# adobe/3D-FM-GAN

Hardware: AMD Instinct MI355X
Metric: (photo,render) pairs/sec (higher is better)
Workload: dtype f32; 1 GPU; pairs1024: cfg4 shard: E_Tsr+E_W+E_W_Plus(18 styles) on 256^2 -> co-mod -> Generator(1024) forward, fp32, B=8/GPU; pairs_per_gpu=8, global_pairs=8, image_size=1024, parallelism=replicas x1 (batch-sharded, no collective), launch=eager, ranks=1, full=False

## Files before the change

3d-fm-gan_amd/op/_native.py:

```python
import ctypes
import os

import torch

_HERE = os.path.dirname(os.path.abspath(__file__))
LIB_PATH = os.environ.get('FMGAN_LIB') or os.path.join(os.path.dirname(_HERE), 'csrc', 'libfmgan_hip.so')

F32, F64, F16 = 0, 1, 2
FMGAN_OK, FMGAN_EUNSUPPORTED = 0, -2
_DTYPES = {torch.float32: F32, torch.float64: F64, torch.float16: F16}

_lib = None

amp_fwd = torch.amp.custom_fwd(device_type='cuda', cast_inputs=torch.float32)
amp_bwd = torch.amp.custom_bwd(device_type='cuda')


def _sig(fn, argtypes, restype=ctypes.c_int):
    fn.argtypes = argtypes
    fn.restype = restype
    return fn


def lib():
    global _lib
    if _lib is not None:
        return _lib
    if not os.path.exists(LIB_PATH):
        raise RuntimeError(
            f'{LIB_PATH} not found: the HIP extension is not built. Run `make -C {os.path.dirname(LIB_PATH)}` '
            f'(or __graft_entry__.build()). There is no CPU or PyTorch fallback for these ops.')
    L = ctypes.CDLL(LIB_PATH)
    vp, i, f, ll = ctypes.c_void_p, ctypes.c_int, ctypes.c_float, ctypes.c_longlong
    _sig(L.fmgan_abi_version, [])
    _sig(L.fmgan_status_string, [i], ctypes.c_char_p)
    _sig(L.fmgan_upfirdn2d_select, [i] * 15)
    _sig(L.fmgan_upfirdn2d_out_size, [i] * 12 + [ctypes.POINTER(i)] * 2)
    _sig(L.fmgan_upfirdn2d, [i, vp, vp, vp] + [i] * 15 + [vp])
    _sig(L.fmgan_upfirdn2d_strided, [i, vp, vp, vp] + [i] * 4 + [ll, i] + [i] * 11 + [vp])
    _sig(L.fmgan_blur_noise_bias_act_f32, [vp] * 3 + [i] * 4 + [ll, i] + [i] * 6 + [vp] * 3 + [i, f, f, vp])
    _sig(L.fmgan_blur_noise_bias_act_select, [vp] * 3 + [i] * 4 + [ll, i] + [i] * 6)
    _sig(L.fmgan_blur_noise_bias_act_path_f32, [vp] * 3 + [i] * 4 + [ll, i] + [i] * 6 + [vp] * 3 + [i, f, f, i, vp])
    _sig(L.fmgan_fused_bias_act, [i, vp, vp, vp, vp, ll, i, i, i, i, f, f, vp])
    _sig(L.fmgan_noise_bias_act_f32, [vp] * 5 + [i] * 4 + [f, f, vp])
    _sig(L.fmgan_fused_bias_act_bwd_blocks, [ll, i])
    _sig(L.fmgan_fused_bias_act_bwd_f32, [vp] * 4 + [ll, i, f, f, vp])
    _sig(L.fmgan_prelu_backward_blocks, [ll, i])
    _sig(L.fmgan_prelu_backward_f32, [vp] * 5 + [ll, i, vp])
    _sig(L.fmgan_face_region_blocks, [i, ll])
    _sig(L.fmgan_face_region_loss_f32, [vp] * 3 + [i, i, ll, vp])
    _sig(L.fmgan_face_region_backward_f32, [vp] * 4 + [i, i, ll, vp])
    _sig(L.fmgan_render_mask_f32, [vp] * 2 + [i, i, ll, vp])
    _sig(L.fmgan_face_input_blocks, [i] * 4)
    _sig(L.fmgan_face_input_f32, [vp] * 5 + [i] * 4 + [vp])
    _sig(L.fmgan_lpips_pair_input_select, [i] * 8)
    _sig(L.fmgan_lpips_pair_input_f32, [vp] * 5 + [i] * 8 + [vp])
    _sig(L.fmgan_projection_loss_select, [i] * 4)
    _sig(L.fmgan_projection_loss_blocks, [i] * 4)
    _sig(L.fmgan_projection_loss_fwd_f32, [vp] * 7 + [i] * 4 + [vp])
    _sig(L.fmgan_projection_loss_bwd_f32, [vp] * 7 + [i] * 4 + [vp])
    _sig(L.fmgan_lpips_distance_blocks, [i] * 3)
    _sig(L.fmgan_lpips_distance_f32, [vp] * 4 + [i, i, i, f, vp])
    _sig(L.fmgan_lpips_distance_backward_f32, [vp] * 6 + [i, i, i, f, vp])
    _sig(L.fmgan_bn_prelu_f32, [vp] * 5 + [f, vp, vp] + [vp] * 4 + [f, vp, vp] + [i] * 5 + [vp])
    _sig(L.fmgan_se_pool_chunks, [i] * 4)
    _sig(L.fmgan_se_pool_f32, [vp, vp] + [i] * 4 + [vp])
    _sig(L.fmgan_se_gate_f32, [vp, i, ll] + [vp] * 4 + [f] + [vp] * 3 + [i] * 3 + [vp])
    _sig(L.fmgan_ir_tail_f32, [vp] * 5 + [f, vp, vp] + [i] * 3 + [vp] * 4 + [f, vp] + [vp] * 4 + [f, vp] + [i] * 4 + [vp])
    _sig(L.fmgan_modconv_demod_f32, [vp] * 3 + [i] * 4 + [f, f, vp])
    _sig(L.fmgan_modconv_wsq_f32, [vp] * 2 + [i] * 3 + [vp])
    _sig(L.fmgan_modconv_demod_wsq_f32, [vp] * 3 + [i] * 3 + [f, f, vp])
    _sig(L.fmgan_equal_linear_f32, [vp] * 4 + [i] * 3 + [vp])
    _sig(L.fmgan_wino_weight_f32, [vp, vp, i, i, vp])
    _sig(L.fmgan_wino_input_f32, [vp] * 3 + [i] * 4 + [vp])
    _sig(L.fmgan_wino_output_f32, [vp] * 6 + [i] * 6 + [f, f, vp])
    _sig(L.fmgan_modconv_weight_prep_f32, [vp, vp, i, i, i, f, i, vp])
    _sig(L.fmgan_modconv2d_workspace_bytes, [i] * 6, ll)
    _sig(L.fmgan_modconv2d_f32, [vp] * 5 + [i] * 6 + [vp] * 3 + [i, i, f, f, ll, i, vp, ll, vp])
    _sig(L.fmgan_modconv_weight_bf16_bytes, [i] * 3, ll)
    _sig(L.fmgan_modconv_weight_to_bf16, [vp, vp, i, i, i, vp])
    _sig(L.fmgan_modconv2d_bf16_supported, [i] * 6)
    _sig(L.fmgan_modconv2d_bf16, [vp] * 5 + [i] * 6 + [vp] * 3 + [i, i, f, f, ll, i, vp])
    _sig(L.fmgan_modconv_weight_bf16x3_bytes, [i] * 3, ll)
    _sig(L.fmgan_modconv_weight_to_bf16x3, [vp, vp, i, i, i, vp])
    _sig(L.fmgan_modconv2d_bf16x3_supported, [i] * 6)
    _sig(L.fmgan_modconv2d_bf16x3, [vp] * 5 + [i] * 6 + [vp] * 3 + [i, i, f, f, ll, i, vp])
    _sig(L.fmgan_modconv2d_rgb_fusable, [i] * 5)
    _sig(L.fmgan_modconv2d_select, [i] * 8 + [ctypes.POINTER(i)] * 5)
    _sig(L.fmgan_modconv2d_tiles, [ctypes.POINTER(i), i])
    _sig(L.fmgan_torgb_weight_mod_f32, [vp] * 3 + [i] * 3 + [f, vp])
    _sig(L.fmgan_modconv2d_rgb_f32, [vp] * 5 + [i] * 5 + [vp] * 3 + [i, i, f, f] + [vp] * 4 + [i, vp])
    _sig(L.fmgan_modconv_wgrad_workspace_bytes, [i] * 5, ll)
    _sig(L.fmgan_modconv_wgrad_f32, [vp] * 5 + [i] * 5 + [f, vp, ll, vp])
    _sig(L.fmgan_modconv_wgrad_mode_workspace_bytes, [i] * 6, ll)
    _sig(L.fmgan_modconv_wgrad_mode_f32, [vp] * 5 + [i] * 6 + [f, vp, ll, vp])
    _sig(L.fmgan_images_to_tensor, [vp, vp, i, i, i, f, f, vp])
    _sig(L.fmgan_resize_output_size, [i, i, i, ctypes.POINTER(ctypes.c_int), ctypes.POINTER(ctypes.c_int)])
    _sig(L.fmgan_resize_plan_ints, [i] * 4, ll)
    _sig(L.fmgan_resize_plan, [i] * 4 + [vp, ll])
    _sig(L.fmgan_resize_bilinear_u8, [vp] * 4 + [i] * 5 + [f, f, vp])
    _sig(L.fmgan_tensor_to_images, [vp, vp, i, i, i, f, f, vp])
    _sig(L.fmgan_torgb_f32, [vp] * 6 + [i] * 4 + [f, vp])
    _sig(L.fmgan_torgb_backward_splits, [i] * 3)
    _sig(L.fmgan_torgb_backward_f32, [vp] * 6 + [i] * 4 + [f, vp])
    _sig(L.fmgan_refresh_entry_bytes, [])
    _sig(L.fmgan_weight_refresh_blocks, [i, i, i, i, ll], ll)
    _sig(L.fmgan_weight_refresh_f32, [vp, i, ll, vp])
    _sig(L.fmgan_style_bank_entry_bytes, [])
    _sig(L.fmgan_style_bank_f32, [vp, i, vp, vp, i, i, i, vp, vp])
    _sig(L.fmgan_demod_bank_f32, [vp, i, vp, i, vp, vp])
    if L.fmgan_abi_version() != 1:
        raise RuntimeError('libfmgan_hip.so ABI version mismatch')
    _lib = L
    return L


def check(status, what):
    if status != FMGAN_OK:
        raise RuntimeError(f'{what}: {lib().fmgan_status_string(status).decode()} (status {status})')


def served(status, what):
    if status == FMGAN_EUNSUPPORTED:
        return False
    check(status, what)
    return True


def require_gpu(t, name):
    if not t.is_cuda:
        raise RuntimeError(f'{name} must be a CUDA tensor (this build has no CPU path)')


def dtype_code(t):
    try:
        return _DTYPES[t.dtype]
    except KeyError:
        raise RuntimeError(f'unsupported dtype {t.dtype}: float32/float64/float16 only') from None


def ptr(t):
    return None if t is None else t.data_ptr()


def fp(t):
    if t is None:
        return None
    if t.dtype != torch.float32 or not t.is_cuda:
        raise RuntimeError(f'libfmgan_hip f32 entry point got a {t.dtype} tensor on {t.device}: float32 GPU tensors only '
                           f'(cast before the call; under autocast the package\'s autograd Functions do)')
    return t.data_ptr()


class on_device:

    def __init__(self, t):
        self.dev = t.device
        self.guard = None

    def __enter__(self):
        if torch.cuda.current_device() != self.dev.index:
            self.guard = torch.cuda.device(self.dev)
            self.guard.__enter__()
        return torch.cuda.current_stream(self.dev).cuda_stream

    def __exit__(self, *exc):
        if self.guard is not None:
            self.guard.__exit__(*exc)
        return False


BLUR_PATHS = {}


class _NullObserver:
    wants_paths = False

    def begin(self, name, info):
        return None

    def end(self, token):
        pass


_observer = _NullObserver()


def set_observer(obs=None):
    global _observer
    _observer = obs if obs is not None else _NullObserver()


class launching(on_device):

    def __init__(self, t, name, info):
        on_device.__init__(self, t)
        self.name, self.info = name, info

    def __enter__(self):
        stream = on_device.__enter__(self)
        self.tok = _observer.begin(self.name, self.info)
        return stream

    def __exit__(self, *exc):
        if exc[0] is None:
            _observer.end(self.tok)
        return on_device.__exit__(self, *exc)


def _noise_args(noise):
    if noise is None:
        return None, 1
    nz = noise.contiguous()
    return nz, nz.shape[0]


def upfirdn2d_out_size(in_h, in_w, kh, kw, up_x, up_y, down_x, down_y, px0, px1, py0, py1):
    oh, ow = ctypes.c_int(), ctypes.c_int()
    check(lib().fmgan_upfirdn2d_out_size(in_h, in_w, kh, kw, up_x, up_y, down_x, down_y, px0, px1, py0, py1,
                                         ctypes.byref(oh), ctypes.byref(ow)), 'upfirdn2d_out_size')
    return oh.value, ow.value
# ... 264 lines not shown

def projection_loss_bwd(x, target, mask, g_y, k, scale):
    b, h, w, f = _projection_loss_args(x, target, mask, (scale,))
    if k.numel() != 1 or k.device != x.device:
        raise ValueError(f'projection_loss_bwd: k must hold one element on x\'s device, got {tuple(k.shape)} on {k.device}')
    if g_y is not None:
        if tuple(g_y.shape) != (b, 3, 256, 256) or not nhwc_dense(g_y) or g_y.device != x.device:
            raise ValueError(f'projection_loss_bwd: g_y {tuple(g_y.shape)} with strides {g_y.stride()}: expected '
                             f'[{b}, 3, 256, 256] in channels_last storage on x\'s device')
    pk, pg = fp(k), fp(g_y)
    if b == 0 or lib().fmgan_projection_loss_select(b, h, w, f) <= 0:
        return None
    with launching(x, 'projection_loss', (b, h, f, mask is not None, g_y is not None, 1)) as stream:
        grad_x = torch.empty_like(x)
        st = lib().fmgan_projection_loss_bwd_f32(fp(x), fp(target), fp(mask), pg, pk, fp(scale), fp(grad_x), b, h, w, f,
                                                 stream)
    return grad_x if served(st, 'projection_loss_bwd') else None


def nhwc_dense(t):
    return t.ndim == 4 and t.permute(0, 2, 3, 1).is_contiguous()


def _lpips_distance_shape(f0, f1, w):
    if f0.ndim != 4 or tuple(f0.shape) != tuple(f1.shape) or w.numel() != f0.shape[1]:
        raise ValueError(f'lpips_distance: features {tuple(f0.shape)} and {tuple(f1.shape)}, weight {tuple(w.shape)}: '
                         f'expected two [N, C, H, W] tensors of one shape and C weights')
    if not (nhwc_dense(f0) and nhwc_dense(f1)):
        raise ValueError('lpips_distance: features must be NHWC-dense (channels_last storage); the kernel reads a '
                         'pixel\'s channel vector as one contiguous run')
    n, c, h, wd = f0.shape
    return n, c, h * wd


def lpips_distance(f0, f1, w, eps=1e-10):
    n, c, hw = _lpips_distance_shape(f0, f1, w)
    w = w.contiguous()
    p0, p1, pw = fp(f0), fp(f1), fp(w)
    if n == 0:
        return torch.zeros((0,), dtype=torch.float32, device=f0.device)
    blocks = lib().fmgan_lpips_distance_blocks(n, c, hw)
    if blocks <= 0:
        return None
    partial = torch.empty((n, blocks), dtype=torch.float32, device=f0.device)
    with launching(f0, 'lpips_distance', (n, c, hw, 0)) as stream:
        st = lib().fmgan_lpips_distance_f32(p0, p1, pw, fp(partial), n, c, hw, float(eps), stream)
    return partial.sum(1) / hw if served(st, 'lpips_distance') else None


def lpips_distance_backward(f0, f1, w, grad, need0, need1, eps=1e-10):
    n, c, hw = _lpips_distance_shape(f0, f1, w)
    if not (need0 or need1):
        return None, None
    gl = grad.reshape(-1)
    if gl.numel() != n:
        raise ValueError(f'lpips_distance_backward: grad must hold one element per sample ({n}), got {tuple(grad.shape)}')
    gl = gl.to(device=f0.device, dtype=torch.float32).contiguous()
    w = w.contiguous()
    p0, p1, pw, pg = fp(f0), fp(f1), fp(w), fp(gl)
    g0 = torch.empty_like(f0) if need0 else None
    g1 = torch.empty_like(f1) if need1 else None
    if n == 0:
        return g0, g1
    with launching(f0, 'lpips_distance', (n, c, hw, 1)) as stream:
        st = lib().fmgan_lpips_distance_backward_f32(p0, p1, pw, pg, fp(g0), fp(g1), n, c, hw, float(eps), stream)
    return (g0, g1) if served(st, 'lpips_distance_backward') else None


def _nhwc(t, name):
    require_gpu(t, name)
    fp(t)
    if not nhwc_dense(t):
        raise RuntimeError(f'{name}: expected a [B,C,H,W] tensor in channels_last storage, got {tuple(t.shape)} with '
                           f'strides {t.stride()}')
    return tuple(t.shape)


def _bn_args(bn, c):
    if bn is None:
        return None, None, None, None, 0.0
    mean, var, gamma, beta, eps = bn
    vs = [v.contiguous() for v in (mean, var, gamma, beta)]
    if any(v.numel() != c for v in vs):
        raise ValueError(f'BatchNorm vectors must hold {c} elements, got {[v.numel() for v in vs]}')
    return fp(vs[0]), fp(vs[1]), fp(vs[2]), fp(vs[3]), float(eps)


def _nhwc_empty(b, c, h, w, device):
    return torch.empty((b, c, h, w), dtype=torch.float32, device=device, memory_format=torch.channels_last)


def bn_prelu(x, bn, slope, want_y=True, bn_next=None, sub_stride=0):
    b, c, h, w = _nhwc(x, 'bn_prelu input')
    if not (want_y or bn_next is not None or sub_stride >= 1):
        raise ValueError('bn_prelu: no output requested')
    slope = slope.contiguous()
    if slope.numel() != c:
        raise ValueError(f'bn_prelu: {slope.numel()} slopes for {c} channels')
    y = torch.empty_like(x) if want_y else None
    y_next = torch.empty_like(x) if bn_next is not None else None
    y_sub = None
    if sub_stride >= 1:
        y_sub = _nhwc_empty(b, c, (h - 1) // sub_stride + 1, (w - 1) // sub_stride + 1, x.device)
    with launching(x, 'bn_prelu', (b, c, h, w)) as stream:
        st = lib().fmgan_bn_prelu_f32(fp(x), *_bn_args(bn, c), fp(slope), fp(y), *_bn_args(bn_next, c), fp(y_next),
                                      fp(y_sub), b, c, h, w, max(int(sub_stride), 0), stream)
    return (y, y_next, y_sub) if served(st, 'bn_prelu') else None


def se_pool(r):
    b, c, h, w = _nhwc(r, 'se_pool input')
    chunks = lib().fmgan_se_pool_chunks(b, c, h, w)
    if chunks <= 0:
        return None
    partial = torch.empty((b, chunks, c), dtype=torch.float32, device=r.device)
    with launching(r, 'se_pool', (b, c, h, w)) as stream:
        st = lib().fmgan_se_pool_f32(fp(r), fp(partial), b, c, h, w, stream)
    return partial if served(st, 'se_pool') else None


def se_gate(partial, hw, bn, fc1, fc2):
    require_gpu(partial, 'se_gate partials')
    b, chunks, c = partial.shape
    mid = fc1.shape[0]
    if tuple(fc1.shape[:2]) != (mid, c) or tuple(fc2.shape[:2]) != (c, mid) or fc1.numel() != mid * c \
            or fc2.numel() != mid * c:
        raise ValueError(f'se_gate: fc1 {tuple(fc1.shape)} / fc2 {tuple(fc2.shape)} do not fit {c} channels')
    fc1, fc2, partial = fc1.reshape(mid, c).contiguous(), fc2.reshape(c, mid).contiguous(), partial.contiguous()
    gate = torch.empty((b, c), dtype=torch.float32, device=partial.device)
    with launching(partial, 'se_gate', (b, c, mid, chunks)) as stream:
        st = lib().fmgan_se_gate_f32(fp(partial), chunks, int(hw), *_bn_args(bn, c), fp(fc1), fp(fc2), fp(gate), b, c,
                                     mid, stream)
    return gate if served(st, 'se_gate') else None


def ir_tail(r, bn, gate, shortcut, sc_stride=1, bn_sc=None, bn_next=None):
    b, c, h, w = _nhwc(r, 'ir_tail input')
    sb, scc, sh, sw = _nhwc(shortcut, 'ir_tail shortcut')
    exp = (h, w) if bn_sc is not None else ((sh - 1) // sc_stride + 1, (sw - 1) // sc_stride + 1)
    if (sb, scc) != (b, c) or exp != (h, w) or (bn_sc is not None and ((sh, sw) != (h, w) or sc_stride != 1)):
        raise ValueError(f'ir_tail: shortcut {tuple(shortcut.shape)} at stride {sc_stride} does not cover {tuple(r.shape)}')
    if gate is not None:
        if tuple(gate.shape) != (b, c):
            raise ValueError(f'ir_tail: gate {tuple(gate.shape)} for {tuple(r.shape)}')
        gate = gate.contiguous()
    out = torch.empty_like(r)
    out_next = torch.empty_like(r) if bn_next is not None else None
    with launching(r, 'ir_tail', (b, c, h, w, sc_stride, bn_sc is not None)) as stream:
        st = lib().fmgan_ir_tail_f32(fp(r), *_bn_args(bn, c), fp(gate), fp(shortcut), sh, sw, int(sc_stride),
                                     *_bn_args(bn_sc, c), fp(out), *_bn_args(bn_next, c), fp(out_next), b, c, h, w, stream)
    return (out, out_next) if served(st, 'ir_tail') else None


def modconv_demod(weight, style, scale, eps=1e-8, wsq=None):
    cout, cin, kh, kw = weight.shape[-4:]
    style = style.contiguous()
    demod = torch.empty((style.shape[0], cout), dtype=torch.float32, device=style.device)
    with on_device(style) as stream:
        if wsq is not None:
            check(lib().fmgan_modconv_demod_wsq_f32(fp(wsq), fp(style), fp(demod), style.shape[0], cout, cin,
                                                    float(scale), float(eps), stream), 'modconv_demod_wsq')
        else:
            check(lib().fmgan_modconv_demod_f32(fp(weight), fp(style), fp(demod), style.shape[0], cout, cin,
                                                kh * kw, float(scale), float(eps), stream), 'modconv_demod')
    return demod


def equal_linear(x, weight, bias=None):
    require_gpu(x, 'input')
    x, weight = x.contiguous(), weight.contiguous()
    b, k = x.shape
    n = weight.shape[0]
    if weight.shape[1] != k:
        raise RuntimeError(f'equal_linear: weight {tuple(weight.shape)} does not match input {tuple(x.shape)}')
    out = torch.empty((b, n), dtype=torch.float32, device=x.device)
    with on_device(x) as stream:
        check(lib().fmgan_equal_linear_f32(fp(x), fp(weight), fp(bias), fp(out), b, n, k, stream), 'equal_linear')
    return out


def style_bank(table, n_entries, w, wplus, styles_out):
    if w.dim() != 2 or wplus.dim() != 3 or wplus.shape[2] != w.shape[1] or not (w.is_contiguous() and wplus.is_contiguous()):
        raise RuntimeError(f'style_bank: W {tuple(w.shape)} / W+ {tuple(wplus.shape)} must be contiguous [T,D] / [P,n,D]')
    with on_device(w) as stream:
        check(lib().fmgan_style_bank_f32(fp(table.view(torch.float32)), n_entries, fp(w), fp(wplus), wplus.shape[0],
                                         w.shape[0], w.shape[1], fp(styles_out), stream), 'style_bank')


def demod_bank(table, n_entries, styles, batch, demod_out):
    with on_device(styles) as stream:
        check(lib().fmgan_demod_bank_f32(fp(table.view(torch.float32)), n_entries, fp(styles), batch, fp(demod_out), stream),
              'demod_bank')


def modconv_wsq(weight):
    cout, cin, kh, kw = weight.shape[-4:]
    wsq = torch.empty((cout, cin), dtype=torch.float32, device=weight.device)
    with on_device(weight) as stream:
        check(lib().fmgan_modconv_wsq_f32(fp(weight), fp(wsq), cout, cin, kh * kw, stream), 'modconv_wsq')
    return wsq


def modconv_weight_prep(weight, scale, kind=0):
    cout, cin, kh, kw = weight.shape[-4:]
    shape = (cin, kh * kw, cout) if kind == 0 else (cout, kh * kw, cin)
    wt = torch.empty(shape, dtype=torch.float32, device=weight.device)
    with on_device(weight) as stream:
        check(lib().fmgan_modconv_weight_prep_f32(fp(weight), fp(wt), cout, cin, kh * kw, float(scale), int(kind),
                                                  stream), 'modconv_weight_prep')
    return wt


def aligned_rows_shape(b, c, oh, ow, pad0):
    off = pad0 % 4
    rs = (ow + off + 31) // 32 * 32
    return (b * c, oh, rs), off, oh * rs, rs


def aligned_rows_buffer(b, c, oh, ow, pad0, device):
    shape, off, ps, rs = aligned_rows_shape(b, c, oh, ow, pad0)
    buf = torch.empty(shape, dtype=torch.float32, device=device)
    return buf, buf.data_ptr() + 4 * off, ps, rs


_mc_precision = 'f32'


class modconv_precision:

    def __init__(self, precision):
        if precision not in ('f32', 'bf16', 'bf16x3'):
            raise ValueError("precision must be 'f32', 'bf16' or 'bf16x3'")
        self.precision = precision

    def __enter__(self):
        global _mc_precision
        self.prev, _mc_precision = _mc_precision, self.precision
        return self

    def __exit__(self, *exc):
        global _mc_precision
        _mc_precision = self.prev
        return False


def modconv_weight_to_bf16(wt):
    cin, taps, cout = wt.shape
    nbytes = lib().fmgan_modconv_weight_bf16_bytes(cin, cout, taps)
    wtb = torch.empty(nbytes // 2, dtype=torch.int16, device=wt.device)
    with on_device(wt) as stream:
        check(lib().fmgan_modconv_weight_to_bf16(fp(wt), ptr(wtb), cin, cout, taps, stream), 'modconv_weight_to_bf16')
    return wtb


def wino_weight(wt):
    cin, taps, cout = wt.shape
    if taps != 9:
        raise RuntimeError('wino_weight: 3x3 weights only')
    u = torch.empty((16, cout, cin), dtype=torch.float32, device=wt.device)
    with on_device(wt) as stream:
        check(lib().fmgan_wino_weight_f32(fp(wt), fp(u), cin, cout, stream), 'wino_weight')
    return u


def wino_input(x, style):
    require_gpu(x, 'input')
    x, style = x.contiguous(), style.contiguous()
    b, cin, h, w = x.shape
    v = torch.empty((16, cin, b * (h // 2) * (w // 2)), dtype=torch.float32, device=x.device)
    with on_device(x) as stream:
        check(lib().fmgan_wino_input_f32(fp(x), fp(style), fp(v), b, cin, h, w, stream), 'wino_input')
    return v


def wino_output(m, demod, batch, h, w, noise=None, noise_weight=None, bias=None, fuse_act=False, alpha=0.2,
                act_scale=2 ** 0.5):
    require_gpu(m, 'm')
    m = m.contiguous()
    cout = m.shape[1]
    if m.shape[0] != 16 or m.shape[2] != batch * (h // 2) * (w // 2):
        raise RuntimeError('wino_output: M must be [16, cout, B*(H/2)*(W/2)]')
    out = torch.empty((batch, cout, h, w), dtype=torch.float32, device=m.device)
    nz, nb = _noise_args(noise)
    with on_device(m) as stream:
        check(lib().fmgan_wino_output_f32(fp(m), fp(demod), fp(nz), fp(noise_weight), fp(bias), fp(out), batch, cout, h, w,
                                          nb, int(bool(fuse_act)), float(alpha), float(act_scale), stream), 'wino_output')
    return out


def modconv2d_winograd(x, wt, style, demod, noise=None, noise_weight=None, bias=None, fuse_act=False, alpha=0.2,
                       act_scale=2 ** 0.5, u=None):
    require_gpu(x, 'input')
    x, style = x.contiguous(), style.contiguous()
    b, cin, h, w = x.shape
    if (h | w) & 1:
        raise RuntimeError('modconv2d_winograd: H and W must be even')
    if u is None:
        u = wino_weight(wt)
    cout = u.shape[1]
    n = b * (h // 2) * (w // 2)
    v = torch.empty((16, cin, n), dtype=torch.float32, device=x.device)
    m = torch.empty((16, cout, n), dtype=torch.float32, device=x.device)
    out = torch.empty((b, cout, h, w), dtype=torch.float32, device=x.device)
    nz, nb = _noise_args(noise)
    with launching(x, 'modconv2d_winograd', (b, cin, cout, h, w, 0)) as stream:
        check(lib().fmgan_wino_input_f32(fp(x), fp(style), fp(v), b, cin, h, w, stream), 'wino_input')
# ... 215 lines not shown
```

3d-fm-gan_amd/psp_encoder_model/encoders/psp_encoders.py:

```python
import math
import os

import torch
import torch.nn.functional as F
from torch import nn
from torch.nn import BatchNorm2d, Conv2d, Module, Sequential

from . import helpers
from .helpers import PReLU, bottleneck_IR, bottleneck_IR_SE, get_blocks
from stylegan2 import EqualLinear
from op import fused_leaky_relu
from op.live_weights import LiveWeights
from Util.streams import overlap_ok, run_deferred, side_streams

HEAD_STREAMS = int(os.environ.get('FMGAN_PSP_STREAMS', '2'))
GROUP_HEADS = os.environ.get('FMGAN_PSP_GROUPED', '0') == '1'

_TAPS = {18: (3, 5, 7), 50: (6, 20, 23)}


class GradualStyleBlock(Module):

    def __init__(self, in_c, out_c, spatial):
        super().__init__()
        self.out_c = out_c
        self.spatial = spatial
        layers, c = [], in_c
        for _ in range(int(math.log2(spatial))):
            layers += [Conv2d(c, out_c, kernel_size=3, stride=2, padding=1), nn.LeakyReLU()]
            c = out_c
        self.convs = nn.Sequential(*layers)
        self.linear = EqualLinear(out_c, out_c, lr_mul=1)

    def forward(self, x):
        if x.is_cuda and x.dtype == torch.float32:
            for conv, act in zip(self.convs[0::2], self.convs[1::2]):
                y = F.conv2d(x, conv.weight, None, conv.stride, conv.padding)
                if y.is_contiguous(memory_format=torch.channels_last) and not y.is_contiguous():
                    n, c, h, w = y.shape
                    y = fused_leaky_relu(y.permute(0, 2, 3, 1).reshape(-1, c), conv.bias, act.negative_slope, 1.0)
                    x = y.view(n, h, w, c).permute(0, 3, 1, 2)
                else:
                    x = fused_leaky_relu(y, conv.bias, act.negative_slope, 1.0)
            return self.linear(x.reshape(-1, self.out_c))
        return self.linear(self.convs(x).reshape(-1, self.out_c))


class GradualStyleEncoder(Module):
    def __init__(self, num_layers, mode='ir', opts=None):
        super().__init__()
        assert num_layers in [18, 50, 100, 152], 'num_layers should be 18, 50, 100, or 152'
        assert mode in ['ir', 'ir_se'], 'mode should be ir or ir_se'
        self.num_layers = num_layers
        unit = bottleneck_IR if mode == 'ir' else bottleneck_IR_SE
        self.input_layer = Sequential(Conv2d(opts.input_nc, 64, (3, 3), 1, 1, bias=False), BatchNorm2d(64), PReLU(64))
        self.body = Sequential(*[unit(b.in_channel, b.depth, b.stride) for stage in get_blocks(num_layers) for b in stage])
        self.style_count = opts.n_styles
        self.coarse_ind = 3
        self.middle_ind = 7
        self.styles = nn.ModuleList()
        for i in range(self.style_count):
            spatial = 16 if i < self.coarse_ind else (32 if i < self.middle_ind else 64)
            self.styles.append(GradualStyleBlock(512, 512, spatial))
        self.latlayer1 = nn.Conv2d(256, 512, kernel_size=1, stride=1, padding=0)
        self.latlayer2 = nn.Conv2d(128, 512, kernel_size=1, stride=1, padding=0)
        self.channels_last = True
        self._cl_key = None
        self._live_weights = None
        self._flat = None

    def _to_channels_last(self):
        w = self.input_layer[0].weight
        key = (w.device, w.data_ptr())
        if self._cl_key != key:
            for m in self.modules():
                if isinstance(m, nn.Conv2d):
                    m.weight.data = m.weight.data.contiguous(memory_format=torch.channels_last)
            self._cl_key = (w.device, self.input_layer[0].weight.data_ptr())

    def _levels(self):
        n = self.style_count
        return [list(range(0, min(self.coarse_ind, n))), list(range(self.coarse_ind, min(self.middle_ind, n))),
                list(range(self.middle_ind, n))]

    def _flatten_heads(self):
        def aliased(big, parts):
            step = big[0:parts[0].shape[0]].numel() * big.element_size()
            return all(q.data_ptr() == big.data_ptr() + g * step and q.stride() == big[0:q.shape[0]].stride()
                       for g, q in enumerate(parts))
        if self._flat is not None and all(aliased(wb, [self.styles[j].convs[2 * d].weight for j in idxs]) and
                                          aliased(bb, [self.styles[j].convs[2 * d].bias for j in idxs])
                                          for idxs, per_depth in self._flat for d, (wb, bb) in enumerate(per_depth)):
            return self._flat
        flat = []
        with torch.no_grad():
            for idxs in self._levels():
                if not idxs:
                    continue
                per_depth = []
                for d in range(len(self.styles[idxs[0]].convs) // 2):
                    convs = [self.styles[j].convs[2 * d] for j in idxs]
                    wb = torch.cat([c.weight.data for c in convs], 0)
                    if convs[0].weight.data.is_contiguous(memory_format=torch.channels_last) and wb.dim() == 4:
                        wb = wb.contiguous(memory_format=torch.channels_last)
                    bb = torch.cat([c.bias.data for c in convs], 0)
                    co = convs[0].weight.shape[0]
                    for g, c in enumerate(convs):
                        c.weight.data = wb[g * co:(g + 1) * co]
                        c.bias.data = bb[g * co:(g + 1) * co]
                    per_depth.append((wb, bb))
                flat.append((idxs, per_depth))
        self._flat = flat
        return flat

    def _grouped_heads(self, level, feat):
        idxs, per_depth = level
        G = len(idxs)
        blocks = [self.styles[j] for j in idxs]
        x = feat
        for d, (wb, bb) in enumerate(per_depth):
            conv, act = blocks[0].convs[2 * d], blocks[0].convs[2 * d + 1]
            y = F.conv2d(x, wb, None, conv.stride, conv.padding, 1, 1 if d == 0 else G)
            n, c, h, w = y.shape
            if y.is_contiguous(memory_format=torch.channels_last) and not y.is_contiguous():
                y = fused_leaky_relu(y.permute(0, 2, 3, 1).reshape(-1, c), bb, act.negative_slope, 1.0)
                x = y.view(n, h, w, c).permute(0, 3, 1, 2)
            else:
                x = fused_leaky_relu(y, bb, act.negative_slope, 1.0)
        out_c = blocks[0].out_c
        xs = x.reshape(-1, G, out_c).transpose(0, 1)
        ws, bs = zip(*[b.linear._scaled_params() for b in blocks])
        out = torch.baddbmm(torch.stack(bs, 0).unsqueeze(1), xs, torch.stack(ws, 0).transpose(1, 2))
        return tuple(out.unbind(0))

    def _upsample_add(self, x, y):
        return F.interpolate(x, size=y.shape[2:], mode='bilinear', align_corners=True) + y

    def forward(self, x):
        heads = self.forward_deferred(x)
        for wait, _ in heads:
            wait()
        return torch.stack([t for _, t in heads], dim=1)

    def forward_deferred(self, x):
        if (not torch.is_grad_enabled()) and x.is_cuda:
            if self._live_weights is None:
                self._live_weights = LiveWeights(self)
            with self._live_weights.fresh():
                return self._forward_deferred(x)
        return self._forward_deferred(x)

    def _forward_deferred(self, x):
        if self.channels_last and x.is_cuda:
            self._to_channels_last()
            x = x.contiguous(memory_format=torch.channels_last)
        t1, t2, t3 = _TAPS[self.num_layers]
        fused = helpers.fused_body(self.input_layer, self.body, x, (t1, t2, t3))
        if fused is not None:
            x, feats = fused
        else:
            x = self.input_layer(x)
            feats = {}
            for i, unit in enumerate(self.body):
                x = unit(x)
                if i in (t1, t2, t3):
                    feats[i] = x
        c1, c2, c3 = feats[t1], feats[t2], feats[t3]
        if GROUP_HEADS and x.is_cuda and x.dtype == torch.float32 and not torch.is_grad_enabled():
            flat = self._flatten_heads()
            if HEAD_STREAMS > 1 and overlap_ok(x):
                streams = side_streams(x.device, HEAD_STREAMS, 'psp-heads')

                def level(k, feat):
                    wait, outs = run_deferred(streams[k % HEAD_STREAMS], self._grouped_heads, flat[k], feat)
                    return [(wait, o) for o in outs]
            else:
                def level(k, feat):
                    return [((lambda: None), o) for o in self._grouped_heads(flat[k], feat)]
            latents = level(0, c3)
            if len(flat) > 1:
                p2 = self._upsample_add(c3, self.latlayer1(c2))
                latents += level(1, p2)
            if len(flat) > 2:
                p1 = self._upsample_add(p2, self.latlayer2(c1))
                latents += level(2, p1)
            return latents
        if HEAD_STREAMS > 1 and overlap_ok(x):
            streams = side_streams(x.device, HEAD_STREAMS, 'psp-heads')

# ... 12 lines not shown
```

include/fmgan_hip.h:

```cpp
#ifndef FMGAN_HIP_H
#define FMGAN_HIP_H

#ifdef __cplusplus
extern "C" {
#endif

#define FMGAN_ABI_VERSION 1

#define FMGAN_OK            0
#define FMGAN_EINVAL       -1
#define FMGAN_EUNSUPPORTED -2
#define FMGAN_ELAUNCH      -3
#define FMGAN_EOVERFLOW    -4

#define FMGAN_F32 0
#define FMGAN_F64 1
#define FMGAN_F16 2

int         fmgan_abi_version(void);
const char *fmgan_status_string(int status);

int fmgan_upfirdn2d_select(int dtype, int major, int in_h, int in_w, int minor,
                           int kernel_h, int kernel_w, int up_x, int up_y,
                           int down_x, int down_y, int pad_x0, int pad_x1,
                           int pad_y0, int pad_y1);

int fmgan_upfirdn2d_out_size(int in_h, int in_w, int kernel_h, int kernel_w,
                             int up_x, int up_y, int down_x, int down_y,
                             int pad_x0, int pad_x1, int pad_y0, int pad_y1,
                             int *out_h, int *out_w);

int fmgan_upfirdn2d(int dtype, const void *input, const void *kernel, void *out,
                    int major, int in_h, int in_w, int minor,
                    int kernel_h, int kernel_w,
                    int up_x, int up_y, int down_x, int down_y,
                    int pad_x0, int pad_x1, int pad_y0, int pad_y1,
                    int force_path, void *stream);

int fmgan_upfirdn2d_strided(int dtype, const void *input, const void *kernel, void *out,
                            int major, int in_h, int in_w, int minor,
                            long long in_plane_stride, int in_row_stride,
                            int kernel_h, int kernel_w,
                            int up_x, int up_y, int down_x, int down_y,
                            int pad_x0, int pad_x1, int pad_y0, int pad_y1,
                            int force_path, void *stream);

int fmgan_blur_noise_bias_act_f32(const float *input, const float *kernel, float *out,
                                  int batch, int channels, int in_h, int in_w,
                                  long long in_plane_stride, int in_row_stride,
                                  int kernel_h, int kernel_w,
                                  int pad_x0, int pad_x1, int pad_y0, int pad_y1,
                                  const float *noise, const float *noise_weight, const float *bias,
                                  int noise_batch, float alpha, float act_scale, void *stream);
int fmgan_blur_noise_bias_act_select(const float *input, const float *out, const float *noise,
                                     int batch, int channels, int in_h, int in_w,
                                     long long in_plane_stride, int in_row_stride,
                                     int kernel_h, int kernel_w,
                                     int pad_x0, int pad_x1, int pad_y0, int pad_y1);
int fmgan_blur_noise_bias_act_path_f32(const float *input, const float *kernel, float *out,
                                       int batch, int channels, int in_h, int in_w,
                                       long long in_plane_stride, int in_row_stride,
                                       int kernel_h, int kernel_w,
                                       int pad_x0, int pad_x1, int pad_y0, int pad_y1,
                                       const float *noise, const float *noise_weight, const float *bias,
                                       int noise_batch, float alpha, float act_scale, int force_path, void *stream);

int fmgan_fused_bias_act(int dtype, const void *x, const void *bias, const void *refer,
                         void *out, long long size_x, int size_b, int step_b,
                         int act, int grad, float alpha, float scale, void *stream);

int fmgan_noise_bias_act_f32(const float *x, const float *noise, const float *noise_weight,
                             const float *bias, float *out,
                             int batch, int channel, int hw, int noise_batch,
                             float alpha, float scale, void *stream);

int fmgan_fused_bias_act_bwd_blocks(long long planes, int hw);
int fmgan_fused_bias_act_bwd_f32(const float *grad_out, const float *ref_out, float *grad_in, float *partial,
                                 long long planes, int hw, float alpha, float scale, void *stream);

int fmgan_prelu_backward_blocks(long long rows, int channels);
int fmgan_prelu_backward_f32(const float *x, const float *grad, const float *slope, float *grad_x,
                             float *partial, long long rows, int channels, void *stream);

int fmgan_face_region_blocks(int batch, long long hw);
int fmgan_face_region_loss_f32(const float *r, const float *g, float *partial, int batch, int channels, long long hw,
                               void *stream);
int fmgan_face_region_backward_f32(const float *r, const float *g, const float *grad_loss, float *grad_g, int batch,
                                   int channels, long long hw, void *stream);
int fmgan_render_mask_f32(const float *r, float *mask, int batch, int channels, long long hw, void *stream);

int fmgan_face_input_blocks(int batch, int h, int w, int k);
int fmgan_face_input_f32(const float *a, const float *b, float *gray_a, float *gray_b, float *l1_partial, int batch,
                         int h, int w, int k, void *stream);

int fmgan_lpips_pair_input_select(int pairs, int h, int w, int y0, int x0, int hc, int wc, int f);
int fmgan_lpips_pair_input_f32(const float *img, const float *shift, const float *scale, float *out0, float *out1,
                               int pairs, int h, int w, int y0, int x0, int hc, int wc, int f, void *stream);

int fmgan_projection_loss_select(int batch, int h, int w, int f);
int fmgan_projection_loss_blocks(int batch, int h, int w, int f);
int fmgan_projection_loss_fwd_f32(const float *x, const float *target, const float *mask, const float *shift,
                                  const float *scale, float *partial, float *y, int batch, int h, int w, int f,
                                  void *stream);
int fmgan_projection_loss_bwd_f32(const float *x, const float *target, const float *mask, const float *g_y,
                                  const float *k, const float *scale, float *grad_x, int batch, int h, int w, int f,
                                  void *stream);

int fmgan_bn_prelu_f32(const float *x, const float *mean, const float *var, const float *gamma, const float *beta,
                       float eps, const float *slope, float *y, const float *next_mean, const float *next_var,
                       const float *next_gamma, const float *next_beta, float next_eps, float *y_next, float *y_sub,
                       int batch, int channels, int h, int w, int sub_stride, void *stream);
int fmgan_se_pool_chunks(int batch, int channels, int h, int w);
int fmgan_se_pool_f32(const float *r, float *partial, int batch, int channels, int h, int w, void *stream);
int fmgan_se_gate_f32(const float *partial, int chunks, long long hw, const float *mean, const float *var,
                      const float *gamma, const float *beta, float eps, const float *fc1, const float *fc2, float *gate,
                      int batch, int channels, int mid, void *stream);
int fmgan_ir_tail_f32(const float *r, const float *mean, const float *var, const float *gamma, const float *beta,
                      float eps, const float *gate, const float *shortcut, int sc_h, int sc_w, int sc_stride,
                      const float *sc_mean, const float *sc_var, const float *sc_gamma, const float *sc_beta, float sc_eps,
                      float *out, const float *next_mean, const float *next_var, const float *next_gamma,
                      const float *next_beta, float next_eps, float *out_next, int batch, int channels, int h, int w,
                      void *stream);

int fmgan_lpips_distance_blocks(int batch, int channels, int hw);
int fmgan_lpips_distance_f32(const float *f0, const float *f1, const float *w, float *partial, int batch, int channels,
                             int hw, float eps, void *stream);
int fmgan_lpips_distance_backward_f32(const float *f0, const float *f1, const float *w, const float *grad,
                                      float *grad_f0, float *grad_f1, int batch, int channels, int hw, float eps,
                                      void *stream);

int fmgan_modconv_demod_f32(const float *weight, const float *style, float *demod,
                            int batch, int cout, int cin, int ktaps,
                            float scale, float eps, void *stream);

int fmgan_wino_weight_f32(const float *wt, float *u, int cin, int cout, void *stream);
int fmgan_wino_input_f32(const float *x, const float *style, float *v, int batch, int c, int h, int w, void *stream);
int fmgan_wino_output_f32(const float *m, const float *demod, const float *noise, const float *noise_weight,
                          const float *bias, float *out, int batch, int cout, int h, int w, int noise_batch,
                          int fuse_act, float alpha, float act_scale, void *stream);

int fmgan_equal_linear_f32(const float *x, const float *weight, const float *bias, float *out,
                           int batch, int n_out, int k_in, void *stream);

int fmgan_modconv_wsq_f32(const float *weight, float *wsq, int cout, int cin, int ktaps, void *stream);
int fmgan_modconv_demod_wsq_f32(const float *wsq, const float *style, float *demod,
                                int batch, int cout, int cin, float scale, float eps, void *stream);

int fmgan_modconv_weight_prep_f32(const float *weight, float *wt, int cout, int cin, int ktaps,
                                  float scale, int kind, void *stream);

typedef struct fmgan_refresh_entry {
  const void *src;
  void *dst;
  void *dst2;
  long long n;
  int kind, cout, cin, ktaps;
  float scale;
  unsigned block_begin;
} fmgan_refresh_entry;
int fmgan_refresh_entry_bytes(void);
long long fmgan_weight_refresh_blocks(int kind, int cout, int cin, int ktaps, long long n);
int fmgan_weight_refresh_f32(const fmgan_refresh_entry *table_dev, int n_entries, long long total_blocks,
                             void *stream);

typedef struct fmgan_style_bank_entry {
  const void *ws;
  const void *bs;
  const void *wsq;
  long long style_off, demod_off;
  int col, sliced, n_styles, cin, cout, demodulate;
  float scale, eps;
} fmgan_style_bank_entry;
int fmgan_style_bank_entry_bytes(void);
int fmgan_style_bank_f32(const fmgan_style_bank_entry *table_dev, int n_entries, const float *w, const float *wplus,
                         int wplus_batch, int batch, int style_dim, float *styles_out, void *stream);
int fmgan_demod_bank_f32(const fmgan_style_bank_entry *table_dev, int n_entries, const float *styles, int batch,
                         float *demod_out, void *stream);

long long fmgan_modconv2d_workspace_bytes(int batch, int cin, int cout, int h, int w, int mode);
int fmgan_modconv2d_f32(const float *in, const float *wt, const float *style,
                        const float *demod, float *out,
                        int batch, int cin, int cout, int h, int w, int mode,
                        const float *noise, const float *noise_weight, const float *bias,
                        int noise_batch, int fuse_act, float alpha, float act_scale,
                        long long out_plane_stride, int out_row_stride,
                        void *workspace, long long workspace_bytes, void *stream);

long long fmgan_modconv_weight_bf16_bytes(int cin, int cout, int ktaps);
int fmgan_modconv_weight_to_bf16(const float *wt, void *wt_bf16, int cin, int cout, int ktaps, void *stream);
int fmgan_modconv2d_bf16_supported(int batch, int cin, int cout, int h, int w, int mode);
int fmgan_modconv2d_bf16(const float *in, const void *wt_bf16, const float *style, const float *demod, float *out,
                         int batch, int cin, int cout, int h, int w, int mode,
                         const float *noise, const float *noise_weight, const float *bias,
                         int noise_batch, int fuse_act, float alpha, float act_scale,
                         long long out_plane_stride, int out_row_stride, void *stream);

long long fmgan_modconv_weight_bf16x3_bytes(int cin, int cout, int ktaps);
int fmgan_modconv_weight_to_bf16x3(const float *wt, void *wt_split, int cin, int cout, int ktaps, void *stream);
int fmgan_modconv2d_bf16x3_supported(int batch, int cin, int cout, int h, int w, int mode);
int fmgan_modconv2d_bf16x3(const float *in, const void *wt_split, const float *style, const float *demod, float *out,
                           int batch, int cin, int cout, int h, int w, int mode,
                           const float *noise, const float *noise_weight, const float *bias,
                           int noise_batch, int fuse_act, float alpha, float act_scale,
                           long long out_plane_stride, int out_row_stride, void *stream);

int fmgan_torgb_weight_mod_f32(const float *rgb_weight, const float *rgb_style, float *wmod,
                               int batch, int cout, int rgb_channels, float rgb_scale, void *stream);
int fmgan_modconv2d_rgb_fusable(int batch, int cin, int cout, int h, int w);
int fmgan_modconv2d_rgb_f32(const float *in, const float *wt, const float *style,
                            const float *demod, float *out,
                            int batch, int cin, int cout, int h, int w,
                            const float *noise, const float *noise_weight, const float *bias,
                            int noise_batch, int fuse_act, float alpha, float act_scale,
                            const float *rgb_wmod, const float *rgb_bias,
                            const float *rgb_skip, float *rgb_out, int rgb_channels, void *stream);

int fmgan_modconv2d_select(int batch, int cin, int cout, int h, int w, int mode, int rgb, int has_workspace,
                           int *cfg, int *variant, int *bm, int *bn, int *ksplit);
int fmgan_modconv2d_tiles(int *out, int cap);

long long fmgan_modconv_wgrad_workspace_bytes(int batch, int cin, int cout, int h, int w);
long long fmgan_modconv_wgrad_mode_workspace_bytes(int batch, int cin, int cout, int h, int w, int mode);
int fmgan_modconv_wgrad_mode_f32(const float *go, const float *demod, const float *x, const float *style,
                                 float *gw, int batch, int cin, int cout, int h, int w, int mode, float scale,
                                 void *workspace, long long workspace_bytes, void *stream);
int fmgan_modconv_wgrad_f32(const float *go, const float *demod, const float *x, const float *style,
                            float *gw, int batch, int cin, int cout, int h, int w, float scale,
                            void *workspace, long long workspace_bytes, void *stream);

int fmgan_torgb_f32(const float *in, const float *weight, const float *style,
                    const float *bias, const float *skip, float *out,
                    int batch, int cin, int cout, int hw, float scale, void *stream);

int fmgan_torgb_backward_splits(int batch, int cin, int hw);
int fmgan_torgb_backward_f32(const float *x, const float *grad_out, const float *weight, const float *style,
                             float *grad_x, float *m_partial, int batch, int cin, int cout, int hw, float scale,
                             void *stream);

int fmgan_resize_output_size(int h, int w, int size, int *out_h, int *out_w);
long long fmgan_resize_plan_ints(int in_h, int in_w, int out_h, int out_w);
int fmgan_resize_plan(int in_h, int in_w, int out_h, int out_w, int *plan, long long plan_ints);
int fmgan_resize_bilinear_u8(const unsigned char *in, const int *plan, unsigned char *out_u8, float *out_f32,
                             int batch, int in_h, int in_w, int out_h, int out_w,
                             float mean, float stdv, void *stream);

int fmgan_images_to_tensor(const unsigned char *in, float *out, int batch, int h, int w,
                           float mean, float stdv, void *stream);
int fmgan_tensor_to_images(const float *in, unsigned char *out, int batch, int h, int w,
                           float cent, float factor, void *stream);

#ifdef __cplusplus
}
#endif
#endif
```

Baseline: 399.9 pairs/s.

## Add split-K MFMA kernel for small pSp style-head convs with fused bias/leaky/linear

Adds a HIP kernel that runs the tiny stride-2 3x3 convolutions in the pSp GradualStyleBlock heads (outputs of 4x4 or smaller) as an implicit GEMM on fp32 MFMA. It splits the K dimension across blocks, using a slab workspace and a ticket counter to pick the block that does the final reduction. Bias and leaky ReLU are fused into the epilogue, and the final 2x2->1x1 conv can chain straight into the equal-linear. The aim is to replace many small, poorly occupied conv2d launches plus separate activation kernels with one better-parallelised launch per layer. The risks are extra workspace allocations per call, ticket-based synchronisation that relies on counters resetting correctly, and the fact that only the last few small layers of each head take this path.

```diff
diff --git a/3d-fm-gan_amd/csrc/psp_heads.hip b/3d-fm-gan_amd/csrc/psp_heads.hip
--- /dev/null
+++ b/3d-fm-gan_amd/csrc/psp_heads.hip
@@ -0,0 +1,208 @@
+#include "common.h"
+
+namespace {
+
+constexpr int kWaves = 8;
+constexpr int kThreads = kWaves * 64;
+constexpr int kChunks = 4;
+constexpr int kMaxSplit = 32;
+constexpr int kMaxRows = 128;
+constexpr int kMaxRowsForced = 2048;
+constexpr int kMaxTickets = 4096;
+
+struct HeadPlan {
+  int mgroups, ntiles, split, ntaps, rows;
+  unsigned long long taps;
+};
+
+bool head_plan(int batch, int ho, int wo, int cin, int cout, int force, HeadPlan* p) {
+  if (ho > 4 || wo > 4) {
+    if (!force || ho > 8 || wo > 8) return false;
+  }
+  if (cin % 8 != 0 || cout % 32 != 0 || cin > 4096 || cout > 4096) return false;
+  const long long rows = (long long)batch * ho * wo;
+  if (rows > (force ? kMaxRowsForced : kMaxRows)) return false;
+  if (rows * 4 * cin >= (1LL << 31)) return false;
+  p->rows = (int)rows;
+  p->mgroups = (int)((rows + 31) / 32);
+  p->ntiles = cout / 32;
+  if (p->ntiles * p->mgroups > kMaxTickets) return false;
+  p->ntaps = 0;
+  p->taps = 0;
+  for (int ky = (ho == 1 ? 1 : 0); ky < 3; ++ky)
+    for (int kx = (wo == 1 ? 1 : 0); kx < 3; ++kx) p->taps |= (unsigned long long)(ky * 3 + kx) << (4 * p->ntaps++);
+  const int steps = p->ntaps * (cin / 8);
+  const int base = p->ntiles * p->mgroups;
+  int split = (FMGAN_NUM_CU + base - 1) / base;
+  const int most = steps / (4 * kWaves) > 1 ? steps / (4 * kWaves) : 1;
+  if (split > most) split = most;
+  if (split > kMaxSplit) split = kMaxSplit;
+  p->split = split;
+  return true;
+}
+
+__device__ __forceinline__ void slab_store(float* p, float v) {
+  __hip_atomic_store(reinterpret_cast<unsigned*>(p), __float_as_uint(v), __ATOMIC_RELAXED, __HIP_MEMORY_SCOPE_AGENT);
+}
+__device__ __forceinline__ float slab_load(const float* p) {
+  return __uint_as_float(__hip_atomic_load(reinterpret_cast<const unsigned*>(p), __ATOMIC_RELAXED, __HIP_MEMORY_SCOPE_AGENT));
+}
+
+struct Operands {
+  f32x4 b[kChunks];
+  f32x4 a[kChunks];
+};
+
+__global__ __launch_bounds__(kThreads) void psp_head_conv_f32(
+    const float* __restrict__ in, const float* __restrict__ wgt, const float* __restrict__ bias,
+    float* __restrict__ out, float* slabs, int* tickets, int h, int w, int ho, int wo, int cin,
+    int cout, int rows, int split, int ntaps, unsigned long long taps, float slope) {
+  __shared__ float red[kWaves - 1][16 * 64];
+  __shared__ int s_last;
+  const int lane = threadIdx.x & 63;
+  const int wave = __builtin_amdgcn_readfirstlane(threadIdx.x >> 6);
+  const int r = lane & 31, hf = lane >> 5;
+  const int n0 = blockIdx.x * 32, m0 = blockIdx.y * 32, s = blockIdx.z;
+  const int c8n = cin >> 3;
+  const int steps = ntaps * c8n;
+  const int kb = (int)((long long)steps * s / split), ke = (int)((long long)steps * (s + 1) / split);
+  const int q0 = kb + (ke - kb) * wave / kWaves, q1 = kb + (ke - kb) * (wave + 1) / kWaves;
+
+  const int m = m0 + r;
+  const bool row_ok = m < rows;
+  const int mm = row_ok ? m : 0;
+  const int bb = mm / (ho * wo), rem = mm - bb * (ho * wo);
+  const int oy = rem / wo, ox = rem - oy * wo;
+  const int rbase = row_ok ? bb * h : -1, roy = 2 * oy - 1, rox = 2 * ox - 1;
+  const float* wrow = wgt + (size_t)(n0 + r) * 9 * cin + 4 * hf;
+  const float* arow = in + 4 * hf;
+
+  f32x16 acc;
+#pragma unroll
+  for (int i = 0; i < 16; ++i) acc[i] = 0.f;
+
+  int ti = q0 / c8n, c8 = q0 - ti * c8n;
+  auto load = [&](Operands& o, int q) {
+#pragma unroll
+    for (int u = 0; u < kChunks; ++u) {
+      if (q + u < q1) {
+        const int tap = (int)((taps >> (4 * ti)) & 15);
+        const int ky = tap / 3, kx = tap - 3 * ky;
+        o.b[u] = *(const f32x4*)(wrow + (size_t)tap * cin + c8 * 8);
+        const int iy = roy + ky, ix = rox + kx;
+        const bool ok = rbase >= 0 && iy >= 0 && iy < h && ix >= 0 && ix < w;
+        f32x4 v = {0.f, 0.f, 0.f, 0.f};
+        if (ok) v = *(const f32x4*)(arow + ((size_t)(rbase + iy) * w + ix) * cin + c8 * 8);
+        o.a[u] = v;
+        if (++c8 == c8n) { c8 = 0; ++ti; }
+      } else {
+        o.b[u] = f32x4{0.f, 0.f, 0.f, 0.f};
+        o.a[u] = f32x4{0.f, 0.f, 0.f, 0.f};
+      }
+    }
+  };
+  auto contract = [&](const Operands& o) {
+#pragma unroll
+    for (int u = 0; u < kChunks; ++u)
+#pragma unroll
+      for (int j = 0; j < 4; ++j) acc = __builtin_amdgcn_mfma_f32_32x32x2f32(o.a[u][j], o.b[u][j], acc, 0, 0, 0);
+  };
+  Operands cur = {}, nxt = {};
+  if (q0 < q1) load(cur, q0);
+  for (int q = q0; q < q1; q += 2 * kChunks) {
+    const bool more = q + kChunks < q1;
+    if (more) load(nxt, q + kChunks);
+    contract(cur);
+    if (more) {
+      if (q + 2 * kChunks < q1) load(cur, q + 2 * kChunks);
+      contract(nxt);
+    }
+  }
+
+  if (wave > 0) {
+#pragma unroll
+    for (int i = 0; i < 16; ++i) red[wave - 1][i * 64 + lane] = acc[i];
+  }
+  __syncthreads();
+  if (wave == 0) {
+#pragma unroll
+    for (int k = 0; k < kWaves - 1; ++k)
+#pragma unroll
+      for (int i = 0; i < 16; ++i) acc[i] += red[k][i * 64 + lane];
+    const float bv = bias[n0 + r];
+#pragma unroll
+    for (int i = 0; i < 16; ++i) {
+      const int mo = m0 + (i & 3) + 8 * (i >> 2) + 4 * hf;
+      if (mo < rows) {
+        if (split == 1) {
+          const float v = acc[i] + bv;
+          out[(size_t)mo * cout + n0 + r] = v > 0.f ? v : v * slope;
+        } else {
+          slab_store(slabs + ((size_t)s * rows + mo) * cout + n0 + r, acc[i]);
+        }
+      }
+    }
+  }
+  if (split == 1) return;
+
+  const int tile = blockIdx.y * gridDim.x + blockIdx.x;
+  if (wave == 0) {
+    asm volatile("s_waitcnt vmcnt(0)" ::: "memory");
+    if (lane == 0)
+      s_last = __hip_atomic_fetch_add(&tickets[tile], 1, __ATOMIC_RELAXED, __HIP_MEMORY_SCOPE_AGENT) == split - 1;
+  }
+  __syncthreads();
+  if (!s_last) return;
+  asm volatile("" ::: "memory");
+  const int nrows = rows - m0 < 32 ? rows - m0 : 32;
+  for (int idx = threadIdx.x; idx < nrows * 32; idx += kThreads) {
+    const size_t off = (size_t)(m0 + (idx >> 5)) * cout + n0 + (idx & 31);
+    float v = 0.f;
+    for (int k0 = 0; k0 < split; k0 += 16) {
+      float p[16];
+#pragma unroll
+      for (int k = 0; k < 16; ++k) p[k] = k0 + k < split ? slab_load(slabs + (size_t)(k0 + k) * rows * cout + off) : 0.f;
+#pragma unroll
+      for (int k = 0; k < 16; ++k) v += p[k];
+    }
+    v += bias[n0 + (idx & 31)];
+    out[off] = v > 0.f ? v : v * slope;
+  }
+  if (threadIdx.x == 0) __hip_atomic_store(&tickets[tile], 0, __ATOMIC_RELAXED, __HIP_MEMORY_SCOPE_AGENT);
+}
+
+inline bool aligned16(const void* p) { return ((uintptr_t)p & 15) == 0; }
+
+}
+extern "C" int fmgan_psp_head_conv_plan(int batch, int h, int w, int cin, int cout, int force, long long* ws_bytes,
+                                        int* n_tickets) {
+  if (batch <= 0 || h <= 0 || w <= 0 || cin <= 0 || cout <= 0) return FMGAN_EINVAL;
+  HeadPlan p;
+  if ((h | w) & 1 || !head_plan(batch, h / 2, w / 2, cin, cout, force, &p)) return FMGAN_EUNSUPPORTED;
+  if (ws_bytes) *ws_bytes = p.split > 1 ? 4LL * p.split * p.rows * cout : 0;
+  if (n_tickets) *n_tickets = p.split > 1 ? p.ntiles * p.mgroups : 0;
+  return FMGAN_OK;
+}
+
+extern "C" int fmgan_psp_head_conv_f32(const float* in, const float* weight, const float* bias, float* out, int batch,
+                                       int h, int w, int cin, int cout, float slope, float* ws, long long ws_bytes,
+                                       void* tickets_dev, int n_tickets, const float* lin_weight, const float* lin_bias,
+                                       float* lin_out, int lin_dim, int force, void* stream) {
+  int* tickets = (int*)tickets_dev;
+  if (batch <= 0 || h <= 0 || w <= 0 || cin <= 0 || cout <= 0) return FMGAN_EINVAL;
+  if (!in || !weight || !bias || !out) return FMGAN_EINVAL;
+  HeadPlan p;
+  if ((h | w) & 1 || !head_plan(batch, h / 2, w / 2, cin, cout, force, &p)) return FMGAN_EUNSUPPORTED;
+  if (!aligned16(in) || !aligned16(weight) || !aligned16(bias) || !aligned16(out) || !aligned16(ws))
+    return FMGAN_EUNSUPPORTED;
+  if (p.split > 1 && (!ws || !tickets || ws_bytes < 4LL * p.split * p.rows * cout || n_tickets < p.ntiles * p.mgroups))
+    return FMGAN_EINVAL;
+  const int ho = h / 2, wo = w / 2;
+  if (lin_weight && (!lin_out || lin_dim <= 0 || ho != 1 || wo != 1)) return FMGAN_EINVAL;
+  const dim3 grid(p.ntiles, p.mgroups, p.split);
+  hipLaunchKernelGGL(psp_head_conv_f32, grid, dim3(kThreads), 0, (hipStream_t)stream, in, weight, bias, out, ws, tickets,
+                     h, w, ho, wo, cin, cout, p.rows, p.split, p.ntaps, p.taps, slope);
+  const int st = fmgan_check_launch();
+  if (st != FMGAN_OK || !lin_weight) return st;
+  return fmgan_equal_linear_f32(out, lin_weight, lin_bias, lin_out, batch, lin_dim, cout, stream);
+}
diff --git a/3d-fm-gan_amd/op/_native.py b/3d-fm-gan_amd/op/_native.py
--- a/3d-fm-gan_amd/op/_native.py
+++ b/3d-fm-gan_amd/op/_native.py
@@ -67,6 +67,8 @@
     _sig(L.fmgan_se_pool_f32, [vp, vp] + [i] * 4 + [vp])
     _sig(L.fmgan_se_gate_f32, [vp, i, ll] + [vp] * 4 + [f] + [vp] * 3 + [i] * 3 + [vp])
     _sig(L.fmgan_ir_tail_f32, [vp] * 5 + [f, vp, vp] + [i] * 3 + [vp] * 4 + [f, vp] + [vp] * 4 + [f, vp] + [i] * 4 + [vp])
+    _sig(L.fmgan_psp_head_conv_plan, [i] * 6 + [vp, ctypes.POINTER(i)])
+    _sig(L.fmgan_psp_head_conv_f32, [vp] * 4 + [i] * 5 + [f, vp, ll, vp, i] + [vp] * 3 + [i, i, vp])
     _sig(L.fmgan_modconv_demod_f32, [vp] * 3 + [i] * 4 + [f, f, vp])
     _sig(L.fmgan_modconv_wsq_f32, [vp] * 2 + [i] * 3 + [vp])
     _sig(L.fmgan_modconv_demod_wsq_f32, [vp] * 3 + [i] * 3 + [f, f, vp])
@@ -637,6 +639,63 @@
     return (out, out_next) if served(st, 'ir_tail') else None
 
 
+_HEAD_PLANS = {}
+_HEAD_TICKETS = {}
+_HEAD_TICKET_INTS = 4096
+
+
+def psp_head_conv_plan(batch, h, w, cin, cout, force=False):
+    key = (batch, h, w, cin, cout, bool(force))
+    try:
+        return _HEAD_PLANS[key]
+    except KeyError:
+        pass
+    plan = None
+    if min(key[:5]) > 0:
+        ws, nt = ctypes.c_longlong(), ctypes.c_int()
+        if served(lib().fmgan_psp_head_conv_plan(batch, h, w, cin, cout, int(bool(force)), ctypes.byref(ws),
+                                                 ctypes.byref(nt)), 'psp_head_conv_plan'):
+            if nt.value > _HEAD_TICKET_INTS:
+                raise RuntimeError(f'psp_head_conv_plan: {nt.value} tickets')
+            plan = (ws.value // 4, nt.value)
+    _HEAD_PLANS[key] = plan
+    return plan
+
+
+def psp_head_conv(x, weight, bias, slope, linear=None, force=False):
+    if not (x.is_cuda and x.dtype == torch.float32 and x.dim() == 4 and weight.dtype == torch.float32
+            and bias is not None and bias.dtype == torch.float32 and weight.dim() == 4 and weight.shape[2:] == (3, 3)
+            and weight.shape[1] == x.shape[1] and weight.device == x.device and bias.device == x.device
+            and x.permute(0, 2, 3, 1).is_contiguous() and weight.permute(0, 2, 3, 1).is_contiguous()
+            and bias.is_contiguous() and bias.numel() == weight.shape[0]):
+        return None
+    b, cin, h, w = x.shape
+    cout = weight.shape[0]
+    plan = psp_head_conv_plan(b, h, w, cin, cout, force)
+    if plan is None:
+        return None
+    lw = lb = lat = None
+    if linear is not None:
+        lw, lb = linear
+        if (h, w) != (2, 2) or lw.dim() != 2 or lw.shape[1] != cout or not lw.is_contiguous() \
+                or (lb is not None and (lb.numel() != lw.shape[0] or not lb.is_contiguous())):
+            raise ValueError(f'psp_head_conv: linear {tuple(lw.shape)} does not follow a {h}x{w} input of {cout} channels')
+    with launching(x, 'psp_head_conv', (b, cin, cout, h, w, linear is not None)) as stream:
+        tk = _HEAD_TICKETS.get((x.device.index, stream))
+        if tk is None:
+            tk = _HEAD_TICKETS[(x.device.index, stream)] = torch.zeros(_HEAD_TICKET_INTS, dtype=torch.int32,
+                                                                        device=x.device)
+        y = _nhwc_empty(b, cout, h // 2, w // 2, x.device)
+        ws = torch.empty(plan[0], dtype=torch.float32, device=x.device) if plan[0] else None
+        if lw is not None:
+            lat = torch.empty((b, lw.shape[0]), dtype=torch.float32, device=x.device)
+        st = lib().fmgan_psp_head_conv_f32(x.data_ptr(), weight.data_ptr(), bias.data_ptr(), y.data_ptr(), b, h, w, cin,
+                                           cout, float(slope), ptr(ws), 4 * plan[0], tk.data_ptr(), _HEAD_TICKET_INTS,
+                                           fp(lw), fp(lb), ptr(lat), 0 if lw is None else lw.shape[0],
+                                           int(bool(force)), stream)
+    return (y, lat) if served(st, 'psp_head_conv') else None
+
+
 def modconv_demod(weight, style, scale, eps=1e-8, wsq=None):
     cout, cin, kh, kw = weight.shape[-4:]
     style = style.contiguous()
diff --git a/3d-fm-gan_amd/psp_encoder_model/encoders/psp_encoders.py b/3d-fm-gan_amd/psp_encoder_model/encoders/psp_encoders.py
--- a/3d-fm-gan_amd/psp_encoder_model/encoders/psp_encoders.py
+++ b/3d-fm-gan_amd/psp_encoder_model/encoders/psp_encoders.py
@@ -9,12 +9,14 @@
 from . import helpers
 from .helpers import PReLU, bottleneck_IR, bottleneck_IR_SE, get_blocks
 from stylegan2 import EqualLinear
-from op import fused_leaky_relu
+from op import fused_leaky_relu, _native
 from op.live_weights import LiveWeights
 from Util.streams import overlap_ok, run_deferred, side_streams
 
 HEAD_STREAMS = int(os.environ.get('FMGAN_PSP_STREAMS', '2'))
 GROUP_HEADS = os.environ.get('FMGAN_PSP_GROUPED', '0') == '1'
+
+HEAD_TAILS = os.environ.get('FMGAN_NO_HEAD_TAILS', '0') != '1'
 
 _TAPS = {18: (3, 5, 7), 50: (6, 20, 23)}
 
@@ -34,7 +36,23 @@
 
     def forward(self, x):
         if x.is_cuda and x.dtype == torch.float32:
-            for conv, act in zip(self.convs[0::2], self.convs[1::2]):
+            tails = (HEAD_TAILS and not torch.is_grad_enabled() and not torch.is_autocast_enabled()
+                     and x.dim() == 4 and x.permute(0, 2, 3, 1).is_contiguous())
+            last = len(self.convs) - 2
+            for k, (conv, act) in enumerate(zip(self.convs[0::2], self.convs[1::2])):
+                if tails and conv.stride == (2, 2) and conv.padding == (1, 1) and _native.psp_head_conv_plan(
+                        x.shape[0], x.shape[2], x.shape[3], x.shape[1], conv.out_channels) is not None:
+                    lin = None
+                    if 2 * k == last and x.shape[2:] == (2, 2) and self.linear.activation is None:
+                        lin = self.linear._scaled_params()
+                        if lin[0].dtype != torch.float32 or not lin[0].is_contiguous():
+                            lin = None
+                    res = _native.psp_head_conv(x, conv.weight, conv.bias, act.negative_slope, lin)
+                    if res is not None:
+                        x, latent = res
+                        if latent is not None:
+                            return latent
+                        continue
                 y = F.conv2d(x, conv.weight, None, conv.stride, conv.padding)
                 if y.is_contiguous(memory_format=torch.channels_last) and not y.is_contiguous():
                     n, c, h, w = y.shape
diff --git a/include/fmgan_hip.h b/include/fmgan_hip.h
--- a/include/fmgan_hip.h
+++ b/include/fmgan_hip.h
@@ -122,6 +122,12 @@
                       const float *next_beta, float next_eps, float *out_next, int batch, int channels, int h, int w,
                       void *stream);
 
+int fmgan_psp_head_conv_plan(int batch, int h, int w, int cin, int cout, int force, long long *ws_bytes, int *n_tickets);
+int fmgan_psp_head_conv_f32(const float *in, const float *weight, const float *bias, float *out, int batch, int h, int w,
+                            int cin, int cout, float slope, float *ws, long long ws_bytes, void *tickets, int n_tickets,
+                            const float *lin_weight, const float *lin_bias, float *lin_out, int lin_dim, int force,
+                            void *stream);
+
 int fmgan_lpips_distance_blocks(int batch, int channels, int hw);
 int fmgan_lpips_distance_f32(const float *f0, const float *f1, const float *w, float *partial, int batch, int channels,
                              int hw, float eps, void *stream);
```

Result: no change. 396.9 pairs/s (-0.7%).
